# SatDump/SatDump

Measured on AMD Instinct MI355X. Metric: Msamples/s IQ through PSK demod -> Viterbi -> RS (HBM-resident cf32), higher is better.
Workload: dtype f32; 1 GPU; metop_ahrpt (BASELINE configs[2]): QPSK 2333333 sym/s @ 6 Msps cf32, conv 3/4-metop, RS(255,223) I=4, 152880 CADUs = 2146959360 samples (17.176 GB) per GPU per step; mode=chunk-parallel (speculate + certify)

## Files before the change

### satdump_amd/csrc/fec_engine.hip

```cpp
#include "m2x_deint.h"
#include "fec_kernels.h"
#include "../../include/sdhip.h"
#include <algorithm>
#include <chrono>
#include <cmath>
#include <functional>
#include <map>
#include <mutex>
#include <vector>

#ifdef SDHIP_HOST_TWIN
constexpr unsigned hipEventDisableTiming = 2;
inline hipError_t hipEventCreateWithFlags(hipEvent_t *e, unsigned) { return hipEventCreate(e); }
inline hipError_t hipStreamWaitEvent(hipStream_t, hipEvent_t, unsigned) { return hipSuccess; }
inline hipError_t hipDeviceGetStreamPriorityRange(int *lo, int *hi)
{
    *lo = *hi = 0;
    return hipSuccess;
}
inline hipError_t hipStreamCreateWithPriority(hipStream_t *s, unsigned flags, int) { return hipStreamCreateWithFlags(s, flags); }
#endif

namespace sdhip
{
// ... 1844 lines not shown
                }
                int accepted = n;
                for (int j = 0; j < n; j++)
                {
                    for (int k = 0; k < 2; k++)
                    {
                        FyRail &r = fy.rail[k];
                        if (dec[k])
                        {
                            const float errors = (float)r.h_io.p[j].ber_err, total = (float)r.h_io.p[j].ber_tot;
                            r.v_ber = (float)((errors / total) * ber_mult);
                            if (r.v_ber > cfg.viterbi_ber_thresold)
                            {
                                r.v_invalid++;
                                if ((float)r.v_invalid > (float)cfg.viterbi_outsync_after)
                                    r.vstate = 0;
                            }
                            else
                                r.v_invalid = 0;
                        }
                        snaps[k][j] = Snap{r.vstate, r.v_invalid, r.v_ber};
                    }
                    if (fy.rail[0].vstate == 0 || fy.rail[1].vstate == 0)
                    {
                        accepted = j + 1;
                        break;
                    }
                }
                int used = accepted;
                if (dec[0] && dec[1])
                {
                    d_vbits.reserve((size_t)accepted * wpb + 4);
                    const FyRail &rx = fy.rail[fy.invert_branches ? 0 : 1], &ry = fy.rail[fy.invert_branches ? 1 : 0];
                    launch_fy_diff(rx.d_vb.p, ry.d_vb.p, accepted, RF, rwpb, fy.x_prev, fy.y_prev, d_vbits.p, wpb, stream);
                    used = deframe_and_emit(accepted, d_out, out_cap_frames, out_written);
                    if (used < accepted)
                        for (int k = 0; k < 2; k++)
                        {
                            fy.rail[k].vstate = snaps[k][used - 1].vstate;
                            fy.rail[k].v_invalid = snaps[k][used - 1].v_invalid;
                            fy.rail[k].v_ber = snaps[k][used - 1].v_ber;
                        }
                    unsigned last[2];
                    SD_HIP(hipMemcpyAsync(&last[0], rx.d_vb.p + (size_t)(used - 1) * rwpb + ((RF - 1) >> 5), 4, hipMemcpyDeviceToHost, stream));
                    SD_HIP(hipMemcpyAsync(&last[1], ry.d_vb.p + (size_t)(used - 1) * rwpb + ((RF - 1) >> 5), 4, hipMemcpyDeviceToHost, stream));
                    SD_HIP(hipStreamSynchronize(stream));
                    fy.x_prev = (last[0] >> (31 - ((RF - 1) & 31))) & 1u;
                    fy.y_prev = (last[1] >> (31 - ((RF - 1) & 31))) & 1u;
                }
                for (int k = 0; k < 2; k++)
                    if (dec[k])
                    {
                        FyRail &r = fy.rail[k];
                        r.dec_first = 0;
                        r.dec_start = r.h_io.p[used - 1].ret_state;
                        r.search.enc_state = (unsigned)r.h_io.p[used - 1].pad;
                    }
                for (int j = 0; j < used; j++)
                    for (int k = 0; k < 2; k++)
                    {
                        const Snap &sn = snaps[k][j];
                        tap_ber.push_back(sn.vstate == 1 ? sn.v_ber : std::min(std::min(10.0f, std::min(fy.rail[k].bers[0], fy.rail[k].bers[1])), std::min(fy.rail[k].bers[2], fy.rail[k].bers[3])));
                        tap_state.push_back(sn.vstate);
                    }
                if (fy.rail[0].vstate == 0 || (!fy.mpt && fy.rail[1].vstate == 0))
                {
                    fy.vit_nosync_run++;
                    stats.watchdog_events++;
                    if (fy.vit_nosync_run >= 10)
                        fy.shift ^= 1;
                }
                pos += used;
                stats.blocks += used;
            }
            stats.viterbi_lock = fy.rail[0].vstate;
            stats.viterbi_ber = fy.rail[0].ber();
            stats.viterbi2_lock = fy.rail[1].vstate;
            stats.viterbi2_ber = fy.rail[1].ber();
            stats.deframer_state = def.state;
            for (int k = 0; k < 8; k++)
                stats.rs_errors[k] = last_errors[k];
        }

        void process_blocks(const int8_t *d_soft, int64_t nblocks, uint8_t *d_out, size_t out_cap_frames, size_t &out_written)
        {
            fence_in();
            if (cfg.decoder == SDHIP_DEC_FENGYUN_AHRPT || cfg.decoder == SDHIP_DEC_FENGYUN_MPT)
                return process_blocks_fengyun(d_soft, nblocks, d_out, out_cap_frames, out_written);
            if (cfg.decoder == SDHIP_DEC_SIMPLE_PSK)
                return process_blocks_simple(d_soft, nblocks, d_out, out_cap_frames, out_written);
            if (punc.rate != 0)
                return process_blocks_punctured(d_soft, nblocks, d_out, out_cap_frames, out_written);
            const bool overlap = env_int("SDHIP_FEC_OVERLAP", 1) != 0;
            hipStream_t sf = overlap ? stream_fwd : stream;
            auto batch_at = [&](int64_t at) -> int {
                const int64_t left = nblocks - at, nb = (left + max_batch - 1) / max_batch;
                return (int)((left + nb - 1) / nb);
            };
            int64_t pos = 0;
            tap_ber.reserve(tap_ber.size() + nblocks);
            tap_state.reserve(tap_state.size() + nblocks);
            int cur = 0;
            int ahead_n = 0;
            try
            {
            while (pos < nblocks)
            {
                if (vstate == 0)
                {
                    run_search(d_soft, pos);
                    if (vstate == 0)
                    {
                        tap_ber.push_back(current_ber());
                        tap_state.push_back(0);
                        pos++;
                        stats.blocks++;
                        continue;
                    }
                    stats.viterbi_lock = 1;
                }
                const bool tdbg = getenv("SDHIP_DEBUG") != nullptr;
                auto t_prev = std::chrono::steady_clock::now();
                auto tick = [&](const char *what) {
                    if (!tdbg)
                        return;
                    const auto t = std::chrono::steady_clock::now();
                    fprintf(stderr, "[sdhip] fec   %-10s %7.3f ms (host wall)\n", what, std::chrono::duration<double, std::milli>(t - t_prev).count());
                    t_prev = t;
                };
                DevBuf<VitBlockIO> &c_dio = cur ? alt.d_io : d_io;
                PinBuf<VitBlockIO> &c_hio = cur ? alt.h_io : h_io;
                DevBuf<uint32_t> &c_vb = cur ? alt.d_vbits : d_vbits;
                Vit2Work &c_w = cur ? alt.vit2 : vit2;
                const bool was_ahead = ahead_n > 0;
                const int n = was_ahead ? ahead_n : batch_at(pos);
                ahead_n = 0;
                if (!was_ahead)
                {
                    vc.iq_swap = v_iq_swap;
                    vc.phase = v_phase;
                    vc.shift = v_shift;
                    vit_issue(vc, d_soft, pos, n, dec_first ? -2 : dec_start, c_dio, c_hio, c_vb, c_w, sf);
                    if (overlap)
                        SD_HIP(hipEventRecord(ev_fwd[cur], sf));
                }
                if (overlap)
                    SD_HIP(hipStreamWaitEvent(stream, ev_fwd[cur], 0));
                int next_n = 0;
                if (overlap && pos + n < nblocks)
                {
                    next_n = batch_at(pos + n);
                    vit_issue(vc, d_soft, pos + n, next_n, -1, cur ? d_io : alt.d_io, cur ? h_io : alt.h_io, cur ? d_vbits : alt.d_vbits, cur ? vit2 : alt.vit2, sf);
                    SD_HIP(hipEventRecord(ev_fwd[cur ^ 1], sf));
                }
                vit_finish(vc, d_soft, pos, n, was_ahead ? dec_start : -1, c_dio, c_hio, c_vb, c_w, search.enc_state, tick);
                int accepted = n;
                const size_t tap0 = tap_ber.size();
                for (int j = 0; j < n; j++)
                {
                    const float errors = (float)c_hio.p[j].ber_err, total = (float)c_hio.p[j].ber_tot;
                    v_ber = (float)((errors / total) * ber_mult);
                    if (v_ber > cfg.viterbi_ber_thresold)
                    {
                        v_invalid++;
                        if ((float)v_invalid > (float)cfg.viterbi_outsync_after)
                            vstate = 0;
                    }
                    else
                        v_invalid = 0;
                    tap_ber.push_back(current_ber());
                    tap_state.push_back(vstate);
                    if (vstate == 0)
                    {
                        accepted = j + 1;
                        break;
                    }
                }
                tick("ber+fsm");
                def_vbits = c_vb.p;
                const int used = deframe_and_emit(accepted, d_out, out_cap_frames, out_written);
                def_vbits = nullptr;
                tick("deframe+rs");
                if (used < accepted)
                {
                    accepted = used;
                    tap_ber.resize(tap0 + accepted);
                    tap_state.resize(tap0 + accepted);
                }
                dec_first = 0;
                dec_start = c_hio.p[accepted - 1].ret_state;
                search.enc_state = (unsigned)c_hio.p[accepted - 1].pad;
                pos += accepted;
                stats.blocks += accepted;
                if (next_n > 0)
                {
                    if (accepted < n || vstate == 0)
                        SD_HIP(hipStreamSynchronize(stream_fwd));
                    else
                    {
                        ahead_n = next_n;
                        cur ^= 1;
                    }
                }
            }
            }
            catch (...)
            {
                def_vbits = nullptr;
                (void)hipStreamSynchronize(stream_fwd);
                (void)hipStreamSynchronize(stream);
                throw;
            }
            stats.viterbi_lock = vstate;
            stats.viterbi_ber = current_ber();
            stats.deframer_state = def.state;
            for (int k = 0; k < 8; k++)
                stats.rs_errors[k] = last_errors[k];
        }

        struct M2xRail
        {
            int vstate = 0, v_iq_swap = 0, v_phase = 0, v_shift = 0, v_invalid = 0;
            float v_ber = 10, v_bers[2][4][2];
            int dec_first = 1, dec_start = 0;
            VitSearchState search{};
            DevBuf<VitSearchState> d_search;
            DevBuf<VitBlockIO> d_io;
            PinBuf<VitBlockIO> h_io;
            DevBuf<uint32_t> d_vb;
            DevBuf<int8_t> d_rail;
            float ber(int nsw, int nph, const int *ph) const
            {
                if (vstate == 1)
                    return v_ber;
                float b = 10;
                for (int s2 = 0; s2 < nsw; s2++)
                    for (int pi = 0; pi < nph; pi++)
                        for (int o = 0; o < 2; o++)
                            if (b > v_bers[s2][ph[pi]][o])
                                b = v_bers[s2][ph[pi]][o];
                return b;
            }
        };
        struct M2x
        {
            M2xBranch br[2];
            M2xRail rail[2];
            DevBuf<int8_t> d_raw, d_raw2;
            long long raw_base = 0, raw_end = 0;
            bool done = false;
            DevBuf<long long> d_pos;
            DevBuf<int> d_ns, d_res;
            DevBuf<unsigned char> d_hard;
            DevBuf<M2xRead> d_reads;
            std::vector<int> which;
            long long iterations = 0;
        } m2x;

        void m2x_init()
        {
            m2x.br[1].second = 1;
            for (M2xRail &r : m2x.rail)
            {
                memset(&r.search, 0, sizeof(r.search));
                r.search.ber_first = 1;
                r.d_search.reserve(1);
                for (auto &a : r.v_bers)
                    for (auto &b2 : a)
                        for (float &c2 : b2)
                            c2 = 10;
            }
        }
        void m2x_append(const int8_t *src, size_t n, bool on_device)
        {
            fence_in();
            long long keep_from = m2x.raw_end;
// ... 652 lines not shown
```

### satdump_amd/csrc/fec_kernels.h

```cpp
#pragma once
#include "common.h"
#include <vector>

namespace sdhip
{
    struct VitCfg
    {
        int mode;
        int B;
        int F;
        int nber;
        int pre_swap;
        int iq_swap;
        int phase;
        int shift;
        int stride;
        int nenc;
        int fy;
    };
    __host__ __device__ inline long long vit_stride(const VitCfg &c) { return c.stride > 0 ? c.stride : c.B; }

    constexpr int VIT_PREPASS = 192;
    constexpr int VIT_TB_OVERLAP = 96;

    struct VitBlockIO
    {
        int start_in;
        int start_used;
        int ret_state;
        int end_state;
        int tb_fallback;
        int ber_err;
        int ber_tot;
        int pad;
    };

    void launch_vit_decode(const VitCfg &cfg, const int8_t *soft, int64_t first_block, int nblk, VitBlockIO *io, uint64_t *decisions, uint32_t *vbits,
                           hipStream_t st, const int *list = nullptr);


    constexpr int VIT2_SEG = 512;
#ifndef SDHIP_VIT2_WARM
#define SDHIP_VIT2_WARM 200
#endif
    constexpr int VIT2_WARM = SDHIP_VIT2_WARM;
    struct Vit2Work
    {
        DevBuf<uint16_t> symu;
        DevBuf<uint64_t> dec;
        DevBuf<uint32_t> specx, endx;
        DevBuf<int> entry, exitst;
    };
    inline bool vit2_supported(const VitCfg &cfg) { return cfg.F >= 2 * VIT2_SEG && cfg.F % VIT2_SEG == 0; }
    enum { VIT2_BOTH = 0, VIT2_FORWARD = 1, VIT2_FINISH = 2 };
    void launch_vit_decode2(const VitCfg &cfg, const int8_t *soft, int64_t first_block, int nblk, VitBlockIO *io, uint32_t *vbits, Vit2Work &w,
                            hipStream_t st, int phase = VIT2_BOTH, int seg_nblk = 0);

    void launch_vit_ber(const VitCfg &cfg, const int8_t *soft, int64_t first_block, int nblk, const uint32_t *vbits, unsigned enc_state_in, VitBlockIO *io,
                        hipStream_t st);

    struct VitSearchState
    {
        int ber_first;
        int ber_start;
        unsigned enc_state;
        uint8_t tail[16];
        int ncand;
        int err[16], tot[16];
    };
    void launch_vit_search(const VitCfg &cfg, const int8_t *soft, int64_t block, int n_swap, const int *phases, int nphases, VitSearchState *d_state,
                           hipStream_t st);

    void launch_fy_rails(const int8_t *soft, int64_t first_block, int nblk, int shift, int invert_second, int8_t *rail0, int8_t *rail1, hipStream_t st, int mpt = 0);
    void launch_fy_diff(const uint32_t *x, const uint32_t *y, int nblk, int bits_per_rail, int wpb_rail, unsigned x_prev, unsigned y_prev, uint32_t *out, int wpb_out,
                        hipStream_t st);

    struct PuncPat
    {
        int n;
        unsigned two;
        unsigned lead128;
        float berscale;
    };
    inline PuncPat punc_pattern(int rate)
    {
        switch (rate)
        {
        case 1:
            return PuncPat{3, 0x02u, 0u, 3.5f};
        case 2:
            return PuncPat{4, 0x0Au, 0u, 5.0f};
        case 3:
            return PuncPat{6, 0x3Au, 0x10u, 8.0f};
        default:
            return PuncPat{8, 0xEEu, 0x40u, 10.0f};
        }
    }
    inline int punc_count(const PuncPat &p, int pos0, int n_in)
    {
        int oo = 0, pos = pos0;
        for (int i = 0; i < n_in; i++)
        {
            oo += ((p.two >> pos) & 1u) ? 2 : 1;
            pos = pos + 1 == p.n ? 0 : pos + 1;
        }
        return oo;
    }
    void launch_punc_static(const VitCfg &c, const int8_t *blk, const PuncPat &pat, int shift, int n_in, unsigned char *out, hipStream_t st);
    void launch_punc_cont(const VitCfg &c, const int8_t *blk, int n_in, const PuncPat &pat, int pos0, int lead, int total, unsigned char *carry,
                          unsigned char *dst, hipStream_t st);
    struct PuncDesc
    {
        int pos0;
        long long off;
    };
    void launch_punc_batch(const VitCfg &c, const int8_t *soft, long long first_block, int nblk, int n_in, const PuncPat &pat, const PuncDesc *desc, unsigned char *lin,
                           hipStream_t st);

    inline int vit_words_per_block(int F)
    {
        int L = (F + 63) / 64;
        L = (L + 31) / 32 * 32;
        return 64 * L / 32;
    }

    struct HardCfg
    {
        int qpsk, nrzm, swap_iq, swap_diff, oqpsk_delay, method2, method3;
        int F;
        long long blocks_done;
        int tail[4];
    };
    void launch_hard_bits(const HardCfg &hc, const int8_t *soft, int nblk, int which, uint32_t *vbits, int wpb, hipStream_t st);

    struct BitStream
    {
        const uint32_t *carry;
// ... 38 lines not shown
```

### satdump_amd/csrc/fec_kernels.hip

```cpp
#include "fec_kernels.h"

namespace sdhip
{
    struct SymFetch
    {
        VitCfg c;
        const int8_t *blk;
        int limit;

        __device__ __forceinline__ unsigned u_at(int j) const
        {
            if (j < 0 || j >= limit)
                return 128u;
            const int q = j & ~1;
            int a = blk[q], b = blk[q + 1];
            if (a == -128)
                a = -127;
            if (b == -128)
                b = -127;
            if (c.pre_swap)
            {
                int t = a;
                a = b;
                b = t;
// ... 1283 lines not shown
#pragma unroll
            for (int r = 0; r < 32; r++)
                endx[(size_t)u * 32 + r] = v2_norm(s, r);
        }
    }

    __global__ __launch_bounds__(64) void k_vit2h_tb(int F, int S, int NSEG, int nblk, const VitBlockIO *io, const uint4 *__restrict__ dec4, long long U64, unsigned *vbits,
                                                      int wpb, int *entry, int *exitst)
    {
        const int u = (int)(blockIdx.x * 64 + threadIdx.x);
        if (u >= nblk * NSEG)
            return;
        const int j = u / NSEG, g = u - j * NSEG;
        const int GPS = S / 8;
        const long long ubase = (long long)j * NSEG;
        auto path = [&](int Gb, unsigned st) -> unsigned {
            int gg = Gb / GPS;
            if (gg > NSEG - 1)
                gg = NSEG - 1;
            const int ql = Gb - gg * GPS;
            unsigned q, byte;
            v2h_where(st, q, byte);
            const unsigned *p = reinterpret_cast<const unsigned *>(dec4 + ((size_t)(ql * 4 + (int)(q >> 2)) * U64 + ubase + gg));
            return ~(p[q & 3u] >> (8u * byte)) & 255u;
        };
        const int Gtop = (g + 1) * GPS, Glow = g * GPS;
        unsigned st;
        if (g == NSEG - 1)
            st = (unsigned)io[j].end_state;
        else
        {
            st = 0u;
            for (int Gb = Gtop + VIT_TB_OVERLAP / 8; Gb > Gtop; Gb--)
                st = v2h_back6(path(Gb, st));
        }
        entry[u] = (int)st;
        unsigned *vb = vbits + (size_t)j * wpb + (size_t)g * (S / 32);
        unsigned long long acc = 0ull;
        for (int Gb = Gtop; Gb >= Glow; Gb--)
        {
            if (Gb == Glow)
                exitst[u] = (int)st;
            const unsigned D = path(Gb, st);
            acc = (acc >> 8) | ((unsigned long long)(__brev(D) >> 24) << 56);
            const int ql = Gb - Glow;
            if ((ql & 3) == 0 && ql < GPS)
                vb[ql >> 2] = (unsigned)(acc >> 26);
            st = v2h_back6(D);
        }
    }

    __global__ __launch_bounds__(64) void k_vit2_cert(int NSEG, int nblk, const unsigned *__restrict__ specx, const unsigned *__restrict__ endx,
                                                       const int *__restrict__ entry, const int *__restrict__ exitst, VitBlockIO *io)
    {
        const int j = (int)(blockIdx.x * 64 + threadIdx.x);
        if (j >= nblk)
            return;
        int fail = 0;
        for (int g = 1; g < NSEG; g++)
        {
            const size_t u = (size_t)j * NSEG + g;
            for (int r = 0; r < 32; r++)
                fail |= specx[u * 32 + r] != endx[(u - 1) * 32 + r];
            fail |= entry[u - 1] != exitst[u];
        }
        io[j].tb_fallback = fail ? 2 : 0;
    }

    void launch_vit_decode2(const VitCfg &cfg, const int8_t *soft, int64_t first_block, int nblk, VitBlockIO *io, uint32_t *vbits, Vit2Work &w, hipStream_t st, int phase,
                            int seg_nblk)
    {
        if (nblk <= 0)
            return;
        const bool do_fwd = phase != VIT2_FINISH, do_fin = phase != VIT2_FORWARD;
        const long long rule_nblk = seg_nblk > 0 ? seg_nblk : nblk;
        const int F = cfg.F;
        int S = VIT2_SEG;
        {
            const char *e = getenv("SDHIP_VIT2_SEG");
            if (e && atoi(e) >= 128 && atoi(e) % 32 == 0 && F % atoi(e) == 0 && F / atoi(e) >= 2)
                S = atoi(e);
            else
                for (int m = 4; m >= 2; m >>= 1)
                    if (F % (m * VIT2_SEG) == 0 && F / (m * VIT2_SEG) >= 2 && rule_nblk * (F / (m * VIT2_SEG)) >= 2 * 65536)
                    {
                        S = m * VIT2_SEG;
                        break;
                    }
        }
        const int NSEG = F / S;
        const int SU = (VIT2_WARM + F + 6 + 8 + 7) / 8 * 8;
        const long long U = (long long)nblk * NSEG, U64 = (U + 63) / 64 * 64;
        if (do_fwd)
        {
            w.dec.reserve((size_t)(S + 8) * U64);
            w.specx.reserve((size_t)U * 32);
            w.endx.reserve((size_t)U * 32);
            w.entry.reserve((size_t)U);
            w.exitst.reserve((size_t)U);
        }
        const int wpb = vit_words_per_block(F);
        const bool hist = !(getenv("SDHIP_VIT2_HIST") && atoi(getenv("SDHIP_VIT2_HIST")) == 0);
        const bool fused = hist && !(getenv("SDHIP_VIT2_FUSED") && atoi(getenv("SDHIP_VIT2_FUSED")) == 0);
        if (!fused && do_fwd)
        {
            w.symu.reserve((size_t)nblk * SU + 64);
            ProfScope _ps("k_vit2_prep", st);
            auto go = [&](auto kern) { hipLaunchKernelGGL(kern, dim3((unsigned)nblk), dim3(256), 0, st, cfg, soft, (long long)first_block, nblk, w.symu.p, SU); };
            static const bool templ = !(getenv("SDHIP_VIT2_PREP_TEMPL") && atoi(getenv("SDHIP_VIT2_PREP_TEMPL")) == 0);
            const int key = (templ && (cfg.mode == 0 || cfg.mode == 1) && cfg.phase >= 0 && cfg.phase <= 3) ? cfg.mode * 4 + cfg.phase : -1;
            switch (key)
            {
            case 0: go(k_vit2_prep<0, 0>); break;
            case 1: go(k_vit2_prep<0, 1>); break;
            case 2: go(k_vit2_prep<0, 2>); break;
            case 3: go(k_vit2_prep<0, 3>); break;
            case 4: go(k_vit2_prep<1, 0>); break;
            case 5: go(k_vit2_prep<1, 1>); break;
            case 6: go(k_vit2_prep<1, 2>); break;
            case 7: go(k_vit2_prep<1, 3>); break;
            default: go(k_vit2_prep<-1, -1>); break;
            }
        }
        if (hist)
        {
            if (do_fwd)
            {
                ProfScope _ps("k_vit2_acs", st);
                auto go = [&](auto kern) {
                    hipLaunchKernelGGL(kern, dim3((unsigned)(U64 / 64)), dim3(64), 0, st, cfg, soft, (long long)first_block, F, S, NSEG, nblk, w.symu.p, SU, io, (uint4 *)w.dec.p, U64, w.specx.p,
                                       w.endx.p);
                };
                const int key = !fused ? -2 : ((cfg.mode == 0 || cfg.mode == 1) && cfg.phase >= 0 && cfg.phase <= 3) ? cfg.mode * 4 + cfg.phase : -1;
                switch (key)
                {
                case 0: go(k_vit2h_acs<0, 0, true>); break;
                case 1: go(k_vit2h_acs<0, 1, true>); break;
                case 2: go(k_vit2h_acs<0, 2, true>); break;
                case 3: go(k_vit2h_acs<0, 3, true>); break;
                case 4: go(k_vit2h_acs<1, 0, true>); break;
                case 5: go(k_vit2h_acs<1, 1, true>); break;
                case 6: go(k_vit2h_acs<1, 2, true>); break;
                case 7: go(k_vit2h_acs<1, 3, true>); break;
                case -1: go(k_vit2h_acs<-1, -1, true>); break;
                default: go(k_vit2h_acs<-1, -1, false>); break;
                }
            }
            if (do_fin)
            {
                ProfScope _ps("k_vit2_tb", st);
                hipLaunchKernelGGL(k_vit2h_tb, dim3((unsigned)(U64 / 64)), dim3(64), 0, st, F, S, NSEG, nblk, io, (const uint4 *)w.dec.p, U64, vbits, wpb, w.entry.p, w.exitst.p);
            }
        }
        else
        {
            if (do_fwd)
            {
                ProfScope _ps("k_vit2_acs", st);
                hipLaunchKernelGGL(k_vit2_acs, dim3((unsigned)(U64 / 64)), dim3(64), 0, st, F, S, NSEG, nblk, w.symu.p, SU, io, (unsigned long long *)w.dec.p, U64,
                                   w.specx.p, w.endx.p);
            }
            if (do_fin)
            {
                ProfScope _ps("k_vit2_tb", st);
                hipLaunchKernelGGL(k_vit2_tb, dim3((unsigned)(U64 / 64)), dim3(64), 0, st, F, S, NSEG, nblk, io, (const unsigned long long *)w.dec.p, U64, vbits, wpb,
                                   w.entry.p, w.exitst.p);
            }
        }
        if (do_fin)
        {
            ProfScope _ps("k_vit2_cert", st);
            hipLaunchKernelGGL(k_vit2_cert, dim3((nblk + 63) / 64), dim3(64), 0, st, NSEG, nblk, w.specx.p, w.endx.p, w.entry.p, w.exitst.p, io);
        }
    }

    __device__ __forceinline__ unsigned getbit(const unsigned *w, int n) { return (w[n >> 5] >> (31 - (n & 31))) & 1u; }

    __device__ __forceinline__ unsigned peek_bits(const unsigned *w, long long off, int n)
    {
        const long long wi = off >> 5;
        const int sh = (int)(off & 31);
        const unsigned long long v = ((unsigned long long)w[wi] << 32) | (unsigned long long)w[wi + 1];
        return (unsigned)((v << sh) >> (64 - n));
    }

    __global__ __launch_bounds__(256) void k_vit_ber(VitCfg c, const int8_t *__restrict__ soft, long long first_block, int nblk, const unsigned *__restrict__ vbits,
                                                      int wpb, unsigned enc_state_in, VitBlockIO *io)
    {
        const int wave = (int)(threadIdx.x >> 6);
        const int lane = lane_id();
        const int j = (int)blockIdx.x * 4 + wave;
        if (j >= nblk)
            return;
        const int nber = c.nber, nenc = c.nenc > 0 ? c.nenc : c.nber;
        const unsigned *vb = vbits + (size_t)j * wpb;
        const unsigned *vprev = (j > 0) ? vbits + (size_t)(j - 1) * wpb : nullptr;
        V2Fetch<-1, -1> fx;
        fx.init(c, soft, first_block, j);
        const int ngroups = (nber + 7) / 8;
        unsigned err = 0, tot = 0;
        for (int gi = lane; gi < ngroups; gi += 64)
        {
            const auto raw = fx.load(VIT2_WARM + 8 * gi);
            const uint4 q = fx.decode(raw);
            const unsigned qq[4] = {q.x, q.y, q.z, q.w};
            const int i0 = 8 * gi;
            unsigned win;
            if (gi > 0)
                win = peek_bits(vb, (long long)i0 - 6, 14);
            else
            {
                const unsigned six = vprev ? peek_bits(vprev, (long long)nenc - 6, 6) : (enc_state_in & 63u);
                win = (six << 8) | peek_bits(vb, 0, 8);
            }
#pragma unroll
            for (int k = 0; k < 8; k++)
            {
                if (i0 + k >= nber)
                    break;
                const unsigned stw = (win >> (7 - k)) & 127u;
                const unsigned o0 = parity32(stw & 79u), o1 = parity32(stw & 109u);
                const unsigned pr = (qq[k >> 1] >> (16 * (k & 1))) & 0xFFFFu;
                const unsigned s0 = pr & 255u, s1 = pr >> 8;
                if (s0 != 128u)
                {
                    tot++;
                    err += ((s0 > 127u) ? 1u : 0u) != o0;
                }
                if (s1 != 128u)
                {
                    tot++;
                    err += ((s1 > 127u) ? 1u : 0u) != o1;
                }
            }
        }
        err = wave_sum_u32(err);
        tot = wave_sum_u32(tot);
        if (lane == 0)
        {
            io[j].ber_err = (int)err;
            io[j].ber_tot = (int)tot;
            unsigned e = 0;
            for (int d = 0; d < 6; d++)
                e |= getbit(vb, nenc - 1 - d) << d;
            io[j].pad = (int)e;
        }
    }

    void launch_vit_ber(const VitCfg &cfg, const int8_t *soft, int64_t first_block, int nblk, const uint32_t *vbits, unsigned enc_state_in, VitBlockIO *io,
                        hipStream_t st)
    {
        if (nblk <= 0)
            return;
        ProfScope _ps("k_vit_ber", st);
        hipLaunchKernelGGL(k_vit_ber, dim3((nblk + 3) / 4), dim3(256), 0, st, cfg, soft, (long long)first_block, nblk, vbits, vit_words_per_block(cfg.F),
                           enc_state_in, io);
    }

    __global__ __launch_bounds__(256) void k_fy_rails(const int8_t *__restrict__ soft, long long first_block, int nblk, int shift, int invert_second, int8_t *rail0,
                                                       int8_t *rail1, int mpt)
    {
        const long long g = (long long)blockIdx.x * 256 + threadIdx.x;
        if (g >= (long long)nblk * 2048)
            return;
        const long long j = g >> 11;
        const int i0 = (int)(g & 2047) * 4;
        const unsigned *w = reinterpret_cast<const unsigned *>(soft + (first_block + j) * 16384);
        unsigned r0 = 0, r1 = 0;
#pragma unroll
        for (int q = 0; q < 4; q++)
        {
            const int p = i0 + q + shift;
            int a = 0, b = 0;
            if (p < 8192)
            {
                const unsigned d = w[p >> 1] >> (16 * (p & 1));
                a = (int)(signed char)(d & 0xffu);
                b = (int)(signed char)((d >> 8) & 0xffu);
                a = a == -128 ? -127 : a;
                b = b == -128 ? -127 : b;
            }
            int v0 = b, v1 = invert_second ? ~a : a;
            int qq = q;
            if (mpt)
            {
                v1 = v1 == -128 ? -127 : v1;
                qq = q ^ 1;
            }
            r0 |= ((unsigned)v0 & 0xffu) << (8 * qq);
            r1 |= ((unsigned)v1 & 0xffu) << (8 * qq);
        }
        reinterpret_cast<unsigned *>(rail0 + j * 8192)[i0 >> 2] = r0;
        reinterpret_cast<unsigned *>(rail1 + j * 8192)[i0 >> 2] = r1;
    }
    void launch_fy_rails(const int8_t *soft, int64_t first_block, int nblk, int shift, int invert_second, int8_t *rail0, int8_t *rail1, hipStream_t st, int mpt)
    {
        if (nblk <= 0)
            return;
        ProfScope _ps("k_fy_rails", st);
        const long long threads = (long long)nblk * 2048;
        hipLaunchKernelGGL(k_fy_rails, dim3((unsigned)((threads + 255) / 256)), dim3(256), 0, st, soft, (long long)first_block, nblk, shift, (invert_second || mpt) ? 1 : 0, rail0, rail1, mpt);
    }

    __global__ __launch_bounds__(256) void k_fy_diff(const unsigned *__restrict__ x, const unsigned *__restrict__ y, int nblk, int bits_per_rail, int wpb_rail,
                                                      unsigned x_prev, unsigned y_prev, unsigned *out, int wpb_out)
    {
        const int wout = 2 * bits_per_rail / 32;
        const long long g = (long long)blockIdx.x * 256 + threadIdx.x;
        if (g >= (long long)nblk * wout)
            return;
        const int j = (int)(g / wout), w = (int)(g - (long long)j * wout);
        const int k0 = 16 * w;
        const unsigned *xb = x + (size_t)j * wpb_rail, *yb = y + (size_t)j * wpb_rail;
        const unsigned xw = xb[k0 >> 5], yw = yb[k0 >> 5];
        unsigned xp, yp;
        if (k0 & 31)
        {
            xp = (xw >> (32 - (k0 & 31))) & 1u;
            yp = (yw >> (32 - (k0 & 31))) & 1u;
        }
        else if (k0 > 0)
        {
            xp = xb[(k0 >> 5) - 1] & 1u;
            yp = yb[(k0 >> 5) - 1] & 1u;
        }
        else if (j > 0)
        {
            xp = (xb - wpb_rail)[(bits_per_rail - 1) >> 5] >> (31 - ((bits_per_rail - 1) & 31)) & 1u;
            yp = (yb - wpb_rail)[(bits_per_rail - 1) >> 5] >> (31 - ((bits_per_rail - 1) & 31)) & 1u;
        }
        else
        {
            xp = x_prev & 1u;
            yp = y_prev & 1u;
        }
        unsigned o = 0;
#pragma unroll
        for (int q = 0; q < 16; q++)
        {
// ... 341 lines not shown
        unsigned out = 0;
        int got = 0;
        while (got < 32)
        {
            const unsigned *base = nullptr;
            long long off = 0, avail = 32;
            if (g < 0)
            {
                avail = -g;
            }
            else if (g < bs.carry_bits)
            {
                base = bs.carry;
                off = g;
                avail = bs.carry_bits - g;
            }
            else
            {
                const long long g2 = g - bs.carry_bits;
                const long long j = g2 / bs.F;
                if (j < bs.nblk)
                {
                    const long long o = g2 - j * bs.F;
                    base = bs.vbits + (size_t)j * bs.wpb;
                    off = o;
                    avail = bs.F - o;
                }
            }
            int take = 32 - got;
            if (avail < take)
                take = (int)avail;
            const unsigned v = base ? peek_bits(base, off, take) : 0u;
            out |= v << (32 - got - take);
            got += take;
            g += take;
        }
        return out;
    }
    __device__ __forceinline__ unsigned stream32(const BitStream &bs, long long g)
    {
        const unsigned r = stream_raw32(bs, g);
        if (!bs.nrzm)
            return r;
        const unsigned prev = stream_raw32(bs, g - 1);
        return r ^ prev;
    }

    __global__ __launch_bounds__(256) void k_sync_search(BitStream bs, long long from, long long total, unsigned asm_sync, unsigned *hits, int hits_cap, int *count)
    {
        const long long i = (long long)blockIdx.x * blockDim.x + threadIdx.x;
        const long long p0 = from + 32 * i;
        if (p0 >= total)
            return;
        const unsigned a = stream32(bs, p0 - 31);
        const unsigned b = stream32(bs, p0 + 1);
        const unsigned long long v = ((unsigned long long)a << 32) | b;
        const unsigned inv = ~asm_sync;
#pragma unroll 4
        for (int k2 = 0; k2 < 32; k2++)
        {
            const long long p = p0 + k2;
            if (p >= total)
                break;
            const unsigned w = (unsigned)(v >> (32 - k2));
            if (w == asm_sync || w == inv)
            {
                const int idx = atomicAdd(count, 1);
                if (idx < hits_cap)
                    hits[idx] = (unsigned)((p - from) << 1) | (w == inv ? 1u : 0u);
            }
        }
    }

    void launch_sync_search(const BitStream &bs, int64_t from, uint32_t asm_sync, uint32_t *hits, int hits_cap, int *count, hipStream_t st)
    {
        const int64_t total = bs.carry_bits + bs.nblk * (int64_t)bs.F;
        const int64_t n = (total - from + 31) / 32;
        if (n <= 0)
            return;
        ProfScope _ps("k_sync_search", st);
        hipLaunchKernelGGL(k_sync_search, dim3((unsigned)((n + 255) / 256)), dim3(256), 0, st, bs, (long long)from, (long long)total, asm_sync, hits, hits_cap, count);
    }

    __global__ __launch_bounds__(256) void k_pack_stream(BitStream bs, unsigned char *out, long long total_bits)
    {
        const long long i = (long long)blockIdx.x * blockDim.x + threadIdx.x;
        if (i * 32 >= total_bits)
            return;
        const unsigned w = stream32(bs, i * 32);
        out[i * 4 + 0] = (unsigned char)(w >> 24);
        out[i * 4 + 1] = (unsigned char)(w >> 16);
        out[i * 4 + 2] = (unsigned char)(w >> 8);
        out[i * 4 + 3] = (unsigned char)(w);
    }
    __global__ __launch_bounds__(256) void k_window_gather(const unsigned char *__restrict__ packed, long long total_bits, long long p0, int step, int K,
                                                            unsigned *words)
    {
        const int k = (int)(blockIdx.x * blockDim.x + threadIdx.x);
        if (k >= K)
            return;
        const long long pk = p0 + (long long)k * step;
#pragma unroll
        for (int o = 0; o < WIN_OFFS; o++)
        {
            const long long p = pk + o;
            unsigned w = 0;
            if (p >= 31 && p < total_bits)
            {
                const long long s0 = p - 31, byte = s0 >> 3;
                const int sh = (int)(s0 & 7);
                unsigned long long v = 0;
                for (int i = 0; i < 5; i++)
                    v = (v << 8) | packed[byte + i];
                w = (unsigned)((v << (24 + sh)) >> 32);
            }
            words[(size_t)k * WIN_OFFS + o] = w;
        }
    }
    void launch_window_gather(const uint8_t *packed, int64_t total_bits, int64_t p0, int step, int K, uint32_t *words, hipStream_t st)
    {
        if (K <= 0)
            return;
        ProfScope _ps("k_window_gather", st);
        hipLaunchKernelGGL(k_window_gather, dim3((K + 255) / 256), dim3(256), 0, st, packed, (long long)total_bits, (long long)p0, step, K, words);
    }
    void launch_pack_stream(const BitStream &bs, uint8_t *out_bytes, int64_t total_bits, hipStream_t st)
    {
        const int64_t n = (total_bits + 31) / 32;
        if (n <= 0)
            return;
        ProfScope _ps("k_pack_stream", st);
        hipLaunchKernelGGL(k_pack_stream, dim3((unsigned)((n + 255) / 256)), dim3(256), 0, st, bs, out_bytes, (long long)total_bits);
    }

    struct GfTables
    {
        unsigned char exp[512];
        unsigned char log[256];
        unsigned char to_dual[256];
        unsigned char from_dual[256];
        unsigned char pn[256];
    };
    static GfTables *g_tables_dev[16] = {nullptr};

    static void build_tables_host(GfTables &t)
    {
        unsigned element = 1;
        t.exp[0] = 1;
        t.log[0] = 0;
        for (unsigned i = 1; i < 512; i++)
        {
            element = element * 2;
            element = (element > 255) ? (element ^ 0x187) : element;
            t.exp[i] = (unsigned char)element;
            if (i < 256)
                t.log[element] = (unsigned char)i;
        }
        auto mul = [&](unsigned a, unsigned b) -> unsigned { return (a == 0 || b == 0) ? 0u : t.exp[t.log[a] + t.log[b]]; };
        for (unsigned x = 0; x < 256; x++)
        {
            unsigned z = 0;
            for (unsigned j = 0; j < 8; j++)
            {
                unsigned y = mul(x, t.exp[(117 * j) % 255]), tr = 0;
                for (int q = 0; q < 8; q++)
                {
                    tr ^= y;
                    y = mul(y, y);
                }
                z |= (tr & 1u) << (7 - j);
            }
            t.to_dual[x] = (unsigned char)z;
        }
        for (unsigned x = 0; x < 256; x++)
            t.from_dual[t.to_dual[x]] = (unsigned char)x;
        unsigned char reg[8] = {1, 1, 1, 1, 1, 1, 1, 1};
        for (int i = 0; i < 255; i++)
        {
            unsigned char byte = 0;
            for (int b = 0; b < 8; b++)
            {
                byte = (unsigned char)(byte << 1 | reg[0]);
                unsigned char nb = reg[0] ^ reg[3] ^ reg[5] ^ reg[7];
                memmove(reg, reg + 1, 7);
                reg[7] = nb;
            }
            t.pn[i] = byte;
        }
        t.pn[255] = 0;
    }

    static const GfTables *tables_for_current_device()
    {
        int dev = 0;
        SD_HIP(hipGetDevice(&dev));
        if (dev < 0 || dev >= 16)
            throw HipError("device ordinal out of range");
        if (!g_tables_dev[dev])
        {
            GfTables h;
            build_tables_host(h);
            GfTables *d = nullptr;
            SD_HIP(hipMalloc((void **)&d, sizeof(GfTables)));
            SD_HIP(hipMemcpy(d, &h, sizeof(GfTables), hipMemcpyHostToDevice));
            g_tables_dev[dev] = d;
        }
        return g_tables_dev[dev];
    }

    struct GfLds
    {
        unsigned char exp[512];
        unsigned char log[256];
    };

// ... 381 lines not shown
            unsigned v = 0;
            if (f0 + fi < nframes && k >= fb && k < 255)
            {
                v = reinterpret_cast<const unsigned *>(data + (size_t)(f0 + fi) * frame_stride)[k - fb];
                if (dualbasis)
                    v = lin8_apply(dual, v);
            }
            stage[fi][k] = v;
        }
        const int fi = tid >> 5, r = tid & 31;
        unsigned S = 0;
        __syncthreads();
        if (r < nroots && f0 + fi < nframes)
        {
            const int fcr = nroots == 32 ? 112 : 120, gap = 11;
            const unsigned lr = (unsigned)((gap * (r + fcr)) % 255);
            const Lin8 mul = lin8_make([&](int x) { return x ? tabs->exp[tabs->log[x] + lr] : (unsigned char)0; });
            const uint4 *row = reinterpret_cast<const uint4 *>(stage[fi]);
#pragma unroll 4
            for (int k4 = 0; k4 < 64; k4++)
            {
                const uint4 q = row[k4];
                S = lin8_apply(mul, S) ^ q.x;
                S = lin8_apply(mul, S) ^ q.y;
                S = lin8_apply(mul, S) ^ q.z;
                if (k4 < 63)
                    S = lin8_apply(mul, S) ^ q.w;
            }
        }
#pragma unroll
        for (int b = 0; b < 4; b++)
            sy_sh[fi * 4 + b][r] = (unsigned char)(S >> (8 * b));
        __syncthreads();
        {
            const int c = tid >> 3, d = tid & 7;
            if (cw0 + c < ncw)
            {
                unsigned char *sp = clean + ((ncw + 15) / 16 * 16) + (size_t)(cw0 + c) * 32;
                reinterpret_cast<unsigned *>(sp)[d] = reinterpret_cast<const unsigned *>(sy_sh[c])[d];
            }
        }
        if (tid < RSS4_FR * 4 && cw0 + tid < ncw)
        {
            unsigned any = 0;
#pragma unroll
            for (int d = 0; d < 8; d++)
                any |= reinterpret_cast<const unsigned *>(sy_sh[tid])[d];
            clean[cw0 + tid] = any ? 0 : 1;
            if (dirty)
            {
                if (any)
                    dirty[1 + atomicAdd(dirty, 1)] = (int)(cw0 + tid);
                else
                    errors[cw0 + tid] = 0;
            }
        }
    }

    void launch_rs_only(uint8_t *data, int nframes, int frame_stride, int dualbasis, int I, int nroots, int fill_bytes, int *errors, hipStream_t st, uint8_t *clean_scratch)
    {
        const long long n = (long long)nframes * I;
        if (n <= 0)
            return;
        const GfTables *tabs = tables_for_current_device();
        int *dirty = nullptr;
        if (clean_scratch)
        {
            dirty = reinterpret_cast<int *>(clean_scratch + rs_scratch_list_offset(n));
            SD_HIP(hipMemsetAsync(dirty, 0, sizeof(int), st));
            ProfScope _ps("k_rs_screen", st);
            static const bool packed_ok = !(getenv("SDHIP_RS_SCREEN4") && atoi(getenv("SDHIP_RS_SCREEN4")) == 0);
            if (packed_ok && I == 4 && frame_stride % 4 == 0 && (reinterpret_cast<uintptr_t>(data) & 3u) == 0)
                hipLaunchKernelGGL(k_rs_screen4, dim3((unsigned)((nframes + RSS4_FR - 1) / RSS4_FR)), dim3(32 * RSS4_FR), 0, st, data, nframes, frame_stride, dualbasis, nroots,
                                   fill_bytes, clean_scratch, tabs, errors, dirty);
            else
                hipLaunchKernelGGL(k_rs_screen, dim3((unsigned)((n + RSS_CW - 1) / RSS_CW)), dim3(32 * RSS_CW), 0, st, data, nframes, frame_stride, dualbasis, I, nroots, fill_bytes,
                                   clean_scratch, tabs, errors, dirty);
        }
        ProfScope _ps("k_rs", st);
        hipLaunchKernelGGL(k_rs, dim3((unsigned)((n + RS_THREADS - 1) / RS_THREADS)), dim3(RS_THREADS), 0, st, data, nframes, frame_stride, dualbasis, I, nroots,
                           fill_bytes, errors, tabs, clean_scratch, dirty);
    }

    __global__ __launch_bounds__(256) void k_extract(BitStream bs, FrameCfg fc, const FrameDesc *frames, int nframes, unsigned char *out, const GfTables *tabs)
    {
        const int f = (int)blockIdx.x;
        if (f >= nframes)
            return;
        const FrameDesc d = frames[f];
        unsigned char *o = out + (size_t)f * fc.cadu_bytes;
        const int nwords = (fc.cadu_bytes + 3) / 4;
        for (int w = (int)threadIdx.x; w < nwords; w += (int)blockDim.x)
        {
            unsigned v;
            if (w == 0)
                v = fc.asm_sync;
            else
            {
                v = stream32(bs, d.pos + (long long)(w - 1) * 32);
                if (d.inv)
                    v = ~v;
            }
            for (int q = 0; q < 4; q++)
            {
                const int k = w * 4 + q;
                if (k >= fc.cadu_bytes)
                    break;
                unsigned byte = (v >> (24 - 8 * q)) & 255u;
                if (fc.derand && !fc.derand_after_rs && k >= fc.derand_start)
                    byte ^= tabs->pn[(k - fc.derand_start) % 255];
                o[k] = (unsigned char)byte;
            }
        }
    }
    __global__ __launch_bounds__(256) void k_derand(unsigned char *frames, int nframes, int cadu_bytes, int derand_start, const GfTables *tabs)
    {
        const long long i = (long long)blockIdx.x * blockDim.x + threadIdx.x;
        if (i >= (long long)nframes * cadu_bytes)
            return;
        const int k = (int)(i % cadu_bytes);
        if (k >= derand_start)
            frames[i] ^= tabs->pn[(k - derand_start) % 255];
    }

    __global__ __launch_bounds__(256) void k_rs_overrun(unsigned char *out, const FrameDesc *frames, int nframes, int cadu_bytes, int I, int dualbasis,
                                                         const int *errors, const GfTables *tabs)
    {
        const int idx = (int)(blockIdx.x * blockDim.x + threadIdx.x);
        const int f = idx >> 2, b = idx & 3;
        if (f + 1 >= nframes || b >= I || !frames[f].pad || errors[(size_t)f * I + b] < 0)
            return;
        const unsigned v = out[(size_t)f * cadu_bytes + 4 + b];
        out[(size_t)(f + 1) * cadu_bytes + b] = dualbasis ? tabs->from_dual[v] : (unsigned char)v;
    }

    void launch_frames(const BitStream &bs, const FrameCfg &fc, const FrameDesc *frames, int nframes, uint8_t *out, int *errors, hipStream_t st, uint8_t *clean_scratch)
    {
        if (nframes <= 0)
            return;
        const GfTables *tabs = tables_for_current_device();
        {
            ProfScope _ps("k_extract", st);
            hipLaunchKernelGGL(k_extract, dim3(nframes), dim3(256), 0, st, bs, fc, frames, nframes, out, tabs);
        }
        if (fc.rs_i != 0)
            launch_rs_only(out + 4, nframes, fc.cadu_bytes, fc.rs_dualbasis, fc.rs_i, fc.rs_nroots, fc.rs_fill_bytes, errors, st, clean_scratch);
        if (fc.rs_i != 0 && fc.rs_fill_bytes == -1 && nframes > 1)
        {
            ProfScope _ps("k_rs_overrun", st);
            hipLaunchKernelGGL(k_rs_overrun, dim3((unsigned)((nframes * 4 + 255) / 256)), dim3(256), 0, st, out, frames, nframes, fc.cadu_bytes, fc.rs_i, fc.rs_dualbasis,
                               errors, tabs);
        }
        if (fc.derand && fc.derand_after_rs)
        {
            const long long n = (long long)nframes * fc.cadu_bytes;
            ProfScope _ps("k_derand", st);
            hipLaunchKernelGGL(k_derand, dim3((unsigned)((n + 255) / 256)), dim3(256), 0, st, out, nframes, fc.cadu_bytes, fc.derand_start, tabs);
        }
    }

    __global__ __launch_bounds__(256) void k_compact(const unsigned char *frames, const int *dst_index, int nframes, int cadu_bytes, unsigned char *out)
    {
        const int f = (int)blockIdx.x;
        if (f >= nframes)
            return;
        const int d = dst_index[f];
        if (d < 0)
            return;
        const unsigned char *s = frames + (size_t)f * cadu_bytes;
        unsigned char *o = out + (size_t)d * cadu_bytes;
        for (int k = (int)threadIdx.x; k < cadu_bytes; k += (int)blockDim.x)
            o[k] = s[k];
    }
    __device__ __forceinline__ bool rs_keep(const int *__restrict__ ferr, int f, int I, int rs_i, int usecheck)
    {
        bool valid = true;
        for (int k = 0; k < rs_i; k++)
            valid = valid && ferr[(size_t)f * I + k] != -1;
        return !usecheck || valid;
    }
    __global__ __launch_bounds__(256) void k_rs_keep(const int *__restrict__ ferr, int nframes, int I, int rs_i, int usecheck, int *wcount)
    {
        const int f = (int)(blockIdx.x * 256 + threadIdx.x);
        const bool keep = f < nframes && rs_keep(ferr, f, I, rs_i, usecheck);
        const unsigned long long m = __ballot(keep);
        if (lane_id() == 0)
            wcount[f >> 6] = __popcll(m);
    }
    __global__ __launch_bounds__(1024) void k_rs_filter(const int *__restrict__ ferr, int nframes, int I, int rs_i, int nwaves, int *wcount, int *info)
    {
        __shared__ int part[1024];
        const int t = (int)threadIdx.x;
        const int per = (nwaves + 1023) / 1024;
        const int a = t * per, b = a + per < nwaves ? a + per : nwaves;
        int c = 0;
        for (int w = a; w < b; w++)
            c += wcount[w];
        part[t] = c;
        __syncthreads();
        for (int off = 1; off < 1024; off <<= 1)
        {
            const int v = t >= off ? part[t - off] : 0;
            __syncthreads();
            part[t] += v;
            __syncthreads();
        }
        int run = part[t] - c;
        for (int w = a; w < b; w++)
        {
            const int n = wcount[w];
            wcount[w] = run;
            run += n;
        }
        if (t == 1023)
            info[0] = part[1023];
        if (t < rs_i && t < 8 && nframes > 0)
            info[1 + t] = ferr[(size_t)(nframes - 1) * I + t];
    }
    __global__ __launch_bounds__(256) void k_rs_slots(const int *__restrict__ ferr, int nframes, int I, int rs_i, int usecheck, int out_base, const int *__restrict__ woff, int *dst)
    {
        const int f = (int)(blockIdx.x * 256 + threadIdx.x);
        const bool keep = f < nframes && rs_keep(ferr, f, I, rs_i, usecheck);
        const unsigned long long m = __ballot(keep);
        const int lane = lane_id();
        const int rank = __popcll(m & ((1ull << lane) - 1ull));
        if (f < nframes)
// ... 22 lines not shown
```

Measured before the change: 57170 Msamples/s.

## Add batch planner and shrink FEC helper kernels to single-wave blocks with dword stores

Replaces the even-split batch sizing with a planner that can split work into batches sized to fill the vit2 long-segment lane threshold, configurable via an environment variable, and resets the plan on rejection. It also changes k_vit_ber, k_pack_stream and k_extract to 64-thread blocks, and replaces byte stores with dword stores (bswap in pack, assembled word in extract). The aim is better batch granularity for the Viterbi path and cheaper memory writes in the framing kernels. Alignment is now required in pack_stream, which throws if the output is unaligned. With PLAN_BATCHES=1 the default plan may match the previous behaviour.

```diff
diff --git a/satdump_amd/csrc/fec_engine.hip b/satdump_amd/csrc/fec_engine.hip
--- a/satdump_amd/csrc/fec_engine.hip
+++ b/satdump_amd/csrc/fec_engine.hip
@@ -1950,6 +1950,49 @@
                 stats.rs_errors[k] = last_errors[k];
         }
 
+        static constexpr int PLAN_BATCHES = 1;
+        std::vector<int> plan_batches(int64_t left) const
+        {
+            const int64_t lmin = (use_vit2 && vit2_supported(vc)) ? vit2_long_segment_blocks(vc) : 0;
+            int64_t nb = lmin > 0 ? std::min<int64_t>(PLAN_BATCHES, left / lmin) : 0, last = 0;
+            if (const char *e = getenv("SDHIP_FEC_PLAN"); e && strchr(e, ':'))
+            {
+                std::vector<int> plan;
+                int64_t n = 1;
+                while (left > 0)
+                {
+                    if (e && atoll(e) >= 1)
+                        n = atoll(e);
+                    e = e && strchr(e, ':') ? strchr(e, ':') + 1 : nullptr;
+                    n = std::min<int64_t>({n, left, max_batch});
+                    plan.push_back((int)n);
+                    left -= n;
+                }
+                return plan;
+            }
+            else if (e)
+            {
+                int en = 0, ed = 0;
+                const int got = sscanf(e, "%d,%d", &en, &ed);
+                if (got >= 1 && en >= 1)
+                    nb = en;
+                if (got == 2 && ed >= 2 && left / ed >= 1)
+                    last = std::min<int64_t>(left / ed, max_batch);
+            }
+            int64_t body = left - last;
+            nb = std::min(std::max<int64_t>({nb, (body + max_batch - 1) / max_batch, 1}), std::max<int64_t>(body, 1));
+            std::vector<int> plan;
+            for (; nb > 0 && body > 0; nb--)
+            {
+                const int64_t n = (body + nb - 1) / nb;
+                plan.push_back((int)n);
+                body -= n;
+            }
+            if (last > 0)
+                plan.push_back((int)last);
+            return plan;
+        }
+
         void process_blocks(const int8_t *d_soft, int64_t nblocks, uint8_t *d_out, size_t out_cap_frames, size_t &out_written)
         {
             fence_in();
@@ -1961,9 +2004,15 @@
                 return process_blocks_punctured(d_soft, nblocks, d_out, out_cap_frames, out_written);
             const bool overlap = env_int("SDHIP_FEC_OVERLAP", 1) != 0;
             hipStream_t sf = overlap ? stream_fwd : stream;
+            std::vector<int> plan;
+            size_t plan_i = 0;
             auto batch_at = [&](int64_t at) -> int {
-                const int64_t left = nblocks - at, nb = (left + max_batch - 1) / max_batch;
-                return (int)((left + nb - 1) / nb);
+                if (plan_i >= plan.size())
+                {
+                    plan = plan_batches(nblocks - at);
+                    plan_i = 0;
+                }
+                return plan[plan_i++];
             };
             int64_t pos = 0;
             tap_ber.reserve(tap_ber.size() + nblocks);
@@ -2060,6 +2109,8 @@
                 search.enc_state = (unsigned)c_hio.p[accepted - 1].pad;
                 pos += accepted;
                 stats.blocks += accepted;
+                if (accepted < n || vstate == 0)
+                    plan.clear();
                 if (next_n > 0)
                 {
                     if (accepted < n || vstate == 0)
diff --git a/satdump_amd/csrc/fec_kernels.h b/satdump_amd/csrc/fec_kernels.h
--- a/satdump_amd/csrc/fec_kernels.h
+++ b/satdump_amd/csrc/fec_kernels.h
@@ -53,6 +53,14 @@
     };
     inline bool vit2_supported(const VitCfg &cfg) { return cfg.F >= 2 * VIT2_SEG && cfg.F % VIT2_SEG == 0; }
     enum { VIT2_BOTH = 0, VIT2_FORWARD = 1, VIT2_FINISH = 2 };
+    constexpr long long VIT2_FILL_LANES = 2 * 65536;
+    inline int vit2_long_segment_blocks(const VitCfg &cfg)
+    {
+        const int S = 4 * VIT2_SEG;
+        if (cfg.F % S != 0 || cfg.F / S < 2)
+            return 0;
+        return (int)((VIT2_FILL_LANES + cfg.F / S - 1) / (cfg.F / S));
+    }
     void launch_vit_decode2(const VitCfg &cfg, const int8_t *soft, int64_t first_block, int nblk, VitBlockIO *io, uint32_t *vbits, Vit2Work &w,
                             hipStream_t st, int phase = VIT2_BOTH, int seg_nblk = 0);
 
diff --git a/satdump_amd/csrc/fec_kernels.hip b/satdump_amd/csrc/fec_kernels.hip
--- a/satdump_amd/csrc/fec_kernels.hip
+++ b/satdump_amd/csrc/fec_kernels.hip
@@ -1389,7 +1389,7 @@
                 S = atoi(e);
             else
                 for (int m = 4; m >= 2; m >>= 1)
-                    if (F % (m * VIT2_SEG) == 0 && F / (m * VIT2_SEG) >= 2 && rule_nblk * (F / (m * VIT2_SEG)) >= 2 * 65536)
+                    if (F % (m * VIT2_SEG) == 0 && F / (m * VIT2_SEG) >= 2 && rule_nblk * (F / (m * VIT2_SEG)) >= VIT2_FILL_LANES)
                     {
                         S = m * VIT2_SEG;
                         break;
@@ -1491,12 +1491,11 @@
         return (unsigned)((v << sh) >> (64 - n));
     }
 
-    __global__ __launch_bounds__(256) void k_vit_ber(VitCfg c, const int8_t *__restrict__ soft, long long first_block, int nblk, const unsigned *__restrict__ vbits,
-                                                      int wpb, unsigned enc_state_in, VitBlockIO *io)
-    {
-        const int wave = (int)(threadIdx.x >> 6);
+    __global__ __launch_bounds__(64) void k_vit_ber(VitCfg c, const int8_t *__restrict__ soft, long long first_block, int nblk, const unsigned *__restrict__ vbits,
+                                                     int wpb, unsigned enc_state_in, VitBlockIO *io)
+    {
         const int lane = lane_id();
-        const int j = (int)blockIdx.x * 4 + wave;
+        const int j = (int)blockIdx.x;
         if (j >= nblk)
             return;
         const int nber = c.nber, nenc = c.nenc > 0 ? c.nenc : c.nber;
@@ -1560,8 +1559,8 @@
         if (nblk <= 0)
             return;
         ProfScope _ps("k_vit_ber", st);
-        hipLaunchKernelGGL(k_vit_ber, dim3((nblk + 3) / 4), dim3(256), 0, st, cfg, soft, (long long)first_block, nblk, vbits, vit_words_per_block(cfg.F),
-                           enc_state_in, io);
+        hipLaunchKernelGGL(k_vit_ber, dim3((unsigned)nblk), dim3(64), 0, st, cfg, soft, (long long)first_block, nblk, vbits, vit_words_per_block(cfg.F), enc_state_in,
+                           io);
     }
 
     __global__ __launch_bounds__(256) void k_fy_rails(const int8_t *__restrict__ soft, long long first_block, int nblk, int shift, int invert_second, int8_t *rail0,
@@ -2069,16 +2068,13 @@
         hipLaunchKernelGGL(k_sync_search, dim3((unsigned)((n + 255) / 256)), dim3(256), 0, st, bs, (long long)from, (long long)total, asm_sync, hits, hits_cap, count);
     }
 
-    __global__ __launch_bounds__(256) void k_pack_stream(BitStream bs, unsigned char *out, long long total_bits)
+    __global__ __launch_bounds__(64) void k_pack_stream(BitStream bs, unsigned char *out, long long total_bits)
     {
         const long long i = (long long)blockIdx.x * blockDim.x + threadIdx.x;
         if (i * 32 >= total_bits)
             return;
         const unsigned w = stream32(bs, i * 32);
-        out[i * 4 + 0] = (unsigned char)(w >> 24);
-        out[i * 4 + 1] = (unsigned char)(w >> 16);
-        out[i * 4 + 2] = (unsigned char)(w >> 8);
-        out[i * 4 + 3] = (unsigned char)(w);
+        reinterpret_cast<unsigned *>(out)[i] = __builtin_bswap32(w);
     }
     __global__ __launch_bounds__(256) void k_window_gather(const unsigned char *__restrict__ packed, long long total_bits, long long p0, int step, int K,
                                                             unsigned *words)
@@ -2116,8 +2112,10 @@
         const int64_t n = (total_bits + 31) / 32;
         if (n <= 0)
             return;
+        if (reinterpret_cast<uintptr_t>(out_bytes) & 3u)
+            throw HipError("launch_pack_stream: the packed stream must start on a dword boundary");
         ProfScope _ps("k_pack_stream", st);
-        hipLaunchKernelGGL(k_pack_stream, dim3((unsigned)((n + 255) / 256)), dim3(256), 0, st, bs, out_bytes, (long long)total_bits);
+        hipLaunchKernelGGL(k_pack_stream, dim3((unsigned)((n + 63) / 64)), dim3(64), 0, st, bs, out_bytes, (long long)total_bits);
     }
 
     struct GfTables
@@ -2665,7 +2663,7 @@
                            fill_bytes, errors, tabs, clean_scratch, dirty);
     }
 
-    __global__ __launch_bounds__(256) void k_extract(BitStream bs, FrameCfg fc, const FrameDesc *frames, int nframes, unsigned char *out, const GfTables *tabs)
+    __global__ __launch_bounds__(64) void k_extract(BitStream bs, FrameCfg fc, const FrameDesc *frames, int nframes, unsigned char *out, const GfTables *tabs)
     {
         const int f = (int)blockIdx.x;
         if (f >= nframes)
@@ -2673,6 +2671,7 @@
         const FrameDesc d = frames[f];
         unsigned char *o = out + (size_t)f * fc.cadu_bytes;
         const int nwords = (fc.cadu_bytes + 3) / 4;
+        const bool dwords = (reinterpret_cast<uintptr_t>(o) & 3u) == 0;
         for (int w = (int)threadIdx.x; w < nwords; w += (int)blockDim.x)
         {
             unsigned v;
@@ -2684,6 +2683,8 @@
                 if (d.inv)
                     v = ~v;
             }
+            const bool whole = dwords && w * 4 + 4 <= fc.cadu_bytes;
+            unsigned le = 0;
             for (int q = 0; q < 4; q++)
             {
                 const int k = w * 4 + q;
@@ -2692,8 +2693,13 @@
                 unsigned byte = (v >> (24 - 8 * q)) & 255u;
                 if (fc.derand && !fc.derand_after_rs && k >= fc.derand_start)
                     byte ^= tabs->pn[(k - fc.derand_start) % 255];
-                o[k] = (unsigned char)byte;
-            }
+                if (whole)
+                    le |= byte << (8 * q);
+                else
+                    o[k] = (unsigned char)byte;
+            }
+            if (whole)
+                reinterpret_cast<unsigned *>(o)[w] = le;
         }
     }
     __global__ __launch_bounds__(256) void k_derand(unsigned char *frames, int nframes, int cadu_bytes, int derand_start, const GfTables *tabs)
@@ -2724,7 +2730,7 @@
         const GfTables *tabs = tables_for_current_device();
         {
             ProfScope _ps("k_extract", st);
-            hipLaunchKernelGGL(k_extract, dim3(nframes), dim3(256), 0, st, bs, fc, frames, nframes, out, tabs);
+            hipLaunchKernelGGL(k_extract, dim3(nframes), dim3(64), 0, st, bs, fc, frames, nframes, out, tabs);
         }
         if (fc.rs_i != 0)
             launch_rs_only(out + 4, nframes, fc.cadu_bytes, fc.rs_dualbasis, fc.rs_i, fc.rs_nroots, fc.rs_fill_bytes, errors, st, clean_scratch);
```

Measured after the change: 57560 Msamples/s, median of 4. Within noise of the previous version (+0.7%).
